# pycompression/python-zlib-ng

Measured on AMD Instinct MI355X. Metric: MB/s compress+decompress, 128 KiB blocks level 6, higher is better.
Workload: dtype u8

## Files before the change

python-zlib-ng_amd/csrc/za_deflate.hip:

```cpp
#include "za_common.h"
#include "za_crc.h"
#include <type_traits>

#define ZA_CH_GROUP 16
#define ZA_CH_OFFS(x) (((x) >> (32 - ZA_HASH_BITS - 2)) & (((1u << ZA_HASH_BITS) - 1u) << 2))
#define ZA_CH_CHUNK (64 * ZA_CH_GROUP)

typedef uint32_t za_v4u32 __attribute__((ext_vector_type(4)));
__device__ __forceinline__ void za_issue_load16(za_v4u32 &dst, const uint8_t *addr)
{
    asm volatile("global_load_dwordx4 %0, %1, off" : "=v"(dst) : "v"(addr) : "memory");
}
template <int NEWER>
__device__ __forceinline__ void za_wait_loads(za_v4u32 &a, za_v4u32 &b, za_v4u32 &c, za_v4u32 &d)
{
    asm volatile("s_waitcnt vmcnt(%4)" : "+v"(a), "+v"(b), "+v"(c), "+v"(d) : "n"(NEWER) : "memory");
}

__device__ __noinline__ uint32_t za_chains_fix(uint32_t h, uint32_t A, uint32_t old, bool ins)
{
    uint32_t near = 0, pre = 0xFFFFFFFFu;
    const int lane = za_lane();
    const unsigned long long insm = __ballot(ins);
    for (int j = 0; j < 64; j++) {
// ... 626 lines not shown
                if (dl != 0 && dl <= L.max_dist && best_len < nice) {
                    const uint32_t q = P - (uint32_t)dl;
                    const uint32_t sh = q & 3u;
                    const uint32_t *cw = (const uint32_t *)(lds + (q & (uint32_t)(ZA_BYTES - 4)));
                    const uint32_t c0 = cw[0], c1 = cw[1], c2 = cw[2], c3 = cw[3], c4 = cw[4];
                    const uint32_t x0 = __builtin_amdgcn_alignbyte(c1, c0, sh) ^ me0, x1 = __builtin_amdgcn_alignbyte(c2, c1, sh) ^ me1;
                    const uint32_t x2 = __builtin_amdgcn_alignbyte(c3, c2, sh) ^ me2, x3 = __builtin_amdgcn_alignbyte(c4, c3, sh) ^ me3;
                    uint32_t fbit, f1, f2, f3;
                    asm("v_ffbl_b32 %0, %4\n\tv_ffbl_b32 %1, %5\n\tv_ffbl_b32 %2, %6\n\tv_ffbl_b32 %3, %7\n\t"
                        "v_add_u32_e64 %1, %1, 32 clamp\n\tv_add_u32_e64 %2, %2, 64 clamp\n\tv_add_u32_e64 %3, %3, %8 clamp\n\t"
                        "v_min3_u32 %0, %0, %1, %2\n\tv_min_u32_e32 %0, %0, %3"
                        : "=&v"(fbit), "=&v"(f1), "=&v"(f2), "=&v"(f3) : "v"(x0), "v"(x1), "v"(x2), "v"(x3), "s"(96u));
                    int len = (int)min(fbit >> 3, 16u);
                    if (len == 16 && cap > 16) len = za_search_extend(win32, q, P, len, maxlen);
                    len = len < cap ? len : cap;
                    const bool better = len > best_len || (len == best_len && dl < best_dist);
                    best_len = better ? len : best_len;
                    best_dist = better ? dl : best_dist;
                }
            }
            uint32_t result = 0;
            if (best_len >= ZA_MIN_MATCH && !(best_len == 3 && best_dist > L.too_far3) && !(best_len == 4 && best_dist > L.too_far4))
                result = ((uint32_t)best_len << 15) | (uint32_t)(best_dist - 1);
            longm = longm || best_len > 64;
            best[p] = __builtin_amdgcn_perm(me0, result, 0x04020100u);
        };
        auto push = [&](bool alive, int p, uint32_t P, uint32_t q, int best_len, int best_dist, int depth) {
            const unsigned long long m = __ballot(alive);
            if (alive) {
                const uint32_t at = wl_n + __builtin_amdgcn_mbcnt_hi((uint32_t)(m >> 32), __builtin_amdgcn_mbcnt_lo((uint32_t)m, 0u));
                wl[2 * at] = (uint32_t)(p - base) | ((uint32_t)best_len << 12) | ((uint32_t)depth << 21);
                wl[2 * at + 1] = (P - q) | ((uint32_t)best_dist << 16);
            }
            wl_n += (uint32_t)__builtin_popcountll(m);
            __builtin_amdgcn_fence(__ATOMIC_RELEASE, "wavefront");
            __builtin_amdgcn_wave_barrier();
        };
        auto batch = [&](uint32_t nb) {
            wl_n -= nb;
            const bool has = (uint32_t)lane < nb;
            uint32_t e0 = 0, e1 = 0;
            __builtin_amdgcn_fence(__ATOMIC_ACQUIRE, "wavefront");
            if (has) { e0 = wl[2 * (wl_n + lane)]; e1 = wl[2 * (wl_n + lane) + 1]; }
            __builtin_amdgcn_fence(__ATOMIC_ACQ_REL, "wavefront");
            __builtin_amdgcn_wave_barrier();
            bool alive = false;
            int p = 0, best_len = 0, best_dist = 0, depth = 0;
            uint32_t P = 0, q = 0;
            if (has) {
                p = base + (int)(e0 & 0xFFFu);
                best_len = (int)((e0 >> 12) & 0x1FFu); depth = (int)(e0 >> 21); best_dist = (int)(e1 >> 16);
                P = goff + (uint32_t)(ZA_WIN + p);
                q = P - (e1 & 0xFFFFu);
                int seg_end = ((p >> sshift) + 1) << sshift;
                if (seg_end > n) seg_end = n;
                int maxlen = seg_end - p;
                if (maxlen > ZA_MAX_MATCH) maxlen = ZA_MAX_MATCH;
                const int cap = L.cap < maxlen ? L.cap : maxlen, nice = L.nice < cap ? L.nice : cap;
                uint32_t me0, me1, me2, me3;
                my16(P, me0, me1, me2, me3);
                const uint32_t sq = q % ZA_RING;
                uint32_t qb = RING_B0 + 2u * sq;
                uint32_t d = *(const uint16_t *)(lds + qb);
                alive = visit(P, me0, me1, me2, me3, maxlen, cap, nice, q, qb, d, best_len, best_dist, depth);
                if (!alive) finish(p, P, me0, me1, me2, me3, maxlen, cap, nice, best_len, best_dist, (uint32_t)linkb[p], USEC ? (uint32_t)linkc[p] : 0u);
            }
            push(alive, p, P, q, best_len, best_dist, depth);
        };
        uint32_t slot = (goff + (uint32_t)(ZA_WIN + base + tid)) % ZA_RING;
        load_own_links(base + ZA_SEARCH_TILE);
#pragma unroll
        for (int k = 0; k < ZA_SEARCH_TILE / ZA_SEARCH_THREADS; k++, slot = slot + ZA_SEARCH_THREADS >= ZA_RING ? slot + ZA_SEARCH_THREADS - ZA_RING : slot + ZA_SEARCH_THREADS) {
            const int p = base + k * ZA_SEARCH_THREADS + tid;
            bool alive = false;
            const uint32_t P = goff + (uint32_t)(ZA_WIN + p);
            uint32_t q = P;
            int best_len = ZA_MIN_MATCH - 1, best_dist = 0, depth = L.chain;
            if (p < n) {
                int seg_end = ((p >> sshift) + 1) << sshift;
                if (seg_end > n) seg_end = n;
                int maxlen = seg_end - p;
                if (maxlen > ZA_MAX_MATCH) maxlen = ZA_MAX_MATCH;
                uint32_t me0, me1, me2, me3;
                my16(P, me0, me1, me2, me3);
                const int cap = L.cap < maxlen ? L.cap : maxlen, nice = L.nice < cap ? L.nice : cap;
                if (maxlen >= ZA_MIN_MATCH) {
                    uint32_t qb = RING_B0 + 2u * slot;
                    uint32_t d = *(const uint16_t *)(lds + qb);
                    alive = visit(P, me0, me1, me2, me3, maxlen, cap, nice, q, qb, d, best_len, best_dist, depth);
                }
                if (!alive) finish(p, P, me0, me1, me2, me3, maxlen, cap, nice, best_len, best_dist, lkb[k], lkc[k]);
            }
            push(alive, p, P, q, best_len, best_dist, depth);
            while (__builtin_amdgcn_readfirstlane((int)wl_n) >= 64) batch(64u);
        }
        for (;;) {
            const uint32_t left = (uint32_t)__builtin_amdgcn_readfirstlane((int)wl_n);
            if (left == 0) break;
            batch(left < 64u ? left : 64u);
        }
        } else {
        uint32_t slot = (goff + (uint32_t)(ZA_WIN + base + (CONSEC ? 4 * tid : tid))) % ZA_RING;
        load_own_links(base + ZA_SEARCH_TILE);
        if (stats && base > 0) stats_issue(base - ZA_SEARCH_TILE);
#ifndef ZA_SEARCH_KUNROLL
#define ZA_SEARCH_KUNROLL 4
#endif
        const int p0c = base + 4 * tid;
        const uint32_t P0c = goff + (uint32_t)(ZA_WIN + p0c);
        uint32_t cm0 = 0, cm1 = 0, cm2 = 0, cm3 = 0, cm4 = 0;
        uint2 cdq = make_uint2(0u, 0u);
        int cseg_end = 0;
        if (CONSEC && p0c < n) {
            const uint32_t w = (P0c & (ZA_BYTES - 1)) >> 2;
            cm0 = win32[w]; cm1 = win32[w + 1]; cm2 = win32[w + 2]; cm3 = win32[w + 3]; cm4 = win32[w + 4];
            cdq = *(const uint2 *)(lds + RING_B0 + 2u * slot);
            cseg_end = ((p0c >> sshift) + 1) << sshift;
            if (cseg_end > n) cseg_end = n;
        }
#pragma unroll
        for (int k = 0; k < ZA_SEARCH_TILE / ZA_SEARCH_THREADS; k++, slot = CONSEC ? slot : slot + ZA_SEARCH_THREADS >= ZA_RING ? slot + ZA_SEARCH_THREADS - ZA_RING : slot + ZA_SEARCH_THREADS) {
            const int p = CONSEC ? p0c + k : base + k * ZA_SEARCH_THREADS + tid;
            res[k] = 0u;
            if (p >= n) continue;
            int seg_end = cseg_end;
            if (!CONSEC) {
                seg_end = ((p >> sshift) + 1) << sshift;
                if (seg_end > n) seg_end = n;
            }
            int maxlen = seg_end - p;
            if (maxlen > ZA_MAX_MATCH) maxlen = ZA_MAX_MATCH;
            uint32_t result = 0;
            const uint32_t P = goff + (uint32_t)(ZA_WIN + p);
            uint32_t me0, me1, me2, me3;
            if (CONSEC) {
                if (k == 0) { me0 = cm0; me1 = cm1; me2 = cm2; me3 = cm3; }
                else {
                    me0 = __builtin_amdgcn_alignbyte(cm1, cm0, (uint32_t)k); me1 = __builtin_amdgcn_alignbyte(cm2, cm1, (uint32_t)k);
                    me2 = __builtin_amdgcn_alignbyte(cm3, cm2, (uint32_t)k); me3 = __builtin_amdgcn_alignbyte(cm4, cm3, (uint32_t)k);
                }
            } else {
                const uint32_t idx = P & (ZA_BYTES - 1), w = idx >> 2, sh = idx & 3u;
                const uint32_t m0 = win32[w], m1 = win32[w + 1], m2 = win32[w + 2], m3 = win32[w + 3], m4 = win32[w + 4];
                me0 = __builtin_amdgcn_alignbyte(m1, m0, sh); me1 = __builtin_amdgcn_alignbyte(m2, m1, sh);
                me2 = __builtin_amdgcn_alignbyte(m3, m2, sh); me3 = __builtin_amdgcn_alignbyte(m4, m3, sh);
            }
            if (maxlen >= ZA_MIN_MATCH) {
                const int cap = L.cap < maxlen ? L.cap : maxlen;
                const int nice = L.nice < cap ? L.nice : cap;
                int best_len = ZA_MIN_MATCH - 1, best_dist = 0;
                uint32_t q = P;
                uint32_t qb = RING_B0 + 2u * (CONSEC ? slot + (uint32_t)k : slot);
                uint32_t d = CONSEC ? ((k < 2 ? cdq.x : cdq.y) >> (16 * (k & 1))) & 0xFFFFu : (uint32_t)*(const uint16_t *)(lds + qb);
                int depth = STEPS > 0 ? STEPS : L.chain;
#pragma unroll
                while (depth-- > 0) {
                    q -= d;
                    qb -= 2u * d;
                    qb += qb < RING_B0 ? RING_BYTES : 0u;
                    const int dist = (int)(P - q);
                    if (dist > L.max_dist) break;
                    d = *(const uint16_t *)(lds + qb);
                    const uint32_t sh = q & 3u;
                    const uint32_t *cw = (const uint32_t *)(lds + (q & (uint32_t)(ZA_BYTES - 4)));
                    const uint32_t c0 = cw[0], c1 = cw[1], c2 = cw[2], c3 = cw[3], c4 = cw[4];
                    uint32_t x0 = __builtin_amdgcn_alignbyte(c1, c0, sh) ^ me0;
                    uint32_t x1 = __builtin_amdgcn_alignbyte(c2, c1, sh) ^ me1;
                    uint32_t x2 = __builtin_amdgcn_alignbyte(c3, c2, sh) ^ me2;
                    uint32_t x3 = __builtin_amdgcn_alignbyte(c4, c3, sh) ^ me3;
                    uint32_t fbit, f1, f2, f3;
                    asm("v_ffbl_b32 %0, %4\n\tv_ffbl_b32 %1, %5\n\tv_ffbl_b32 %2, %6\n\tv_ffbl_b32 %3, %7\n\t"
                        "v_add_u32_e64 %1, %1, 32 clamp\n\tv_add_u32_e64 %2, %2, 64 clamp\n\tv_add_u32_e64 %3, %3, %8 clamp\n\t"
                        "v_min3_u32 %0, %0, %1, %2\n\tv_min_u32_e32 %0, %0, %3"
                        : "=&v"(fbit), "=&v"(f1), "=&v"(f2), "=&v"(f3) : "v"(x0), "v"(x1), "v"(x2), "v"(x3), "s"(96u));
                    int len = (int)min(fbit >> 3, FULL ? 16u : (uint32_t)cap);
                    if (FULL && len == 16 && cap > 16 && best_len < cap &&
                        (best_len < 16 || (uint8_t)za_lds_ld32(win32, q + (uint32_t)best_len) == (uint8_t)za_lds_ld32(win32, P + (uint32_t)best_len))) {
                        len = za_search_extend(win32, q, P, len, maxlen);
                    }
                    if (FULL) len = len < cap ? len : cap;
                    const bool better = len > best_len;
                    best_len = better ? len : best_len;
                    best_dist = better ? dist : best_dist;
                    if (best_len >= nice) break;
                }
                bool from_bc = false;
#ifndef ZA_ABL_SEARCH_NO_B
                {
                    const uint32_t dl = lkb[k];
#ifdef ZA_ABL_BC_SELF
                    const uint32_t q2 = P - (dl & 3u);
#else
                    const uint32_t q2 = P - dl;
#endif
                    const uint32_t *cw = (const uint32_t *)(lds + (q2 & (uint32_t)(ZA_BYTES - 4)));
                    const uint32_t c0 = cw[0], c1 = cw[1];
                    const uint32_t x = (__builtin_amdgcn_alignbyte(c1, c0, q2 & 3u) ^ me0) << 8;
                    const bool better = x == 0u && dl != 0u && (int)dl <= L.max_dist &&
                                        (ZA_HASH_BYTES_B > best_len || (ZA_HASH_BYTES_B == best_len && (int)dl < best_dist));
                    best_len = better ? ZA_HASH_BYTES_B : best_len;
                    best_dist = better ? (int)dl : best_dist;
                    from_bc = better;
                }
#endif
#ifndef ZA_ABL_SEARCH_NO_C
                if (USEC) {
                    const uint32_t dl = lkc[k];
#ifdef ZA_ABL_BC_SELF
                    const uint32_t q2 = P - (dl & 3u);
#else
                    const uint32_t q2 = P - dl;
#endif
                    const uint32_t sh = q2 & 3u;
                    const uint32_t *cw = (const uint32_t *)(lds + (q2 & (uint32_t)(ZA_BYTES - 4)));
                    const uint32_t c0 = cw[0], c1 = cw[1], c2 = cw[2], c3 = cw[3];
                    const uint32_t x = (__builtin_amdgcn_alignbyte(c1, c0, sh) ^ me0) | (__builtin_amdgcn_alignbyte(c2, c1, sh) ^ me1) |
                                       (__builtin_amdgcn_alignbyte(c3, c2, sh) ^ me2);
                    const bool better = x == 0u && dl != 0u && (int)dl <= L.max_dist && cap >= ZA_HASH_BYTES_C &&
                                        (ZA_HASH_BYTES_C > best_len || (ZA_HASH_BYTES_C == best_len && (int)dl < best_dist));
                    best_len = better ? ZA_HASH_BYTES_C : best_len;
                    best_dist = better ? (int)dl : best_dist;
                    from_bc = from_bc || better;
                }
#endif
#ifndef ZA_ABL_NO_EXTEND
                if (!FULL && (best_len == cap || from_bc) && best_len < maxlen) {
                    best_len = za_search_extend(win32, P - (uint32_t)best_dist, P, best_len, maxlen);
                }
#endif
                if (best_len >= ZA_MIN_MATCH && !(best_len == 3 && best_dist > L.too_far3) && !(best_len == 4 && best_dist > L.too_far4))
                    result = ((uint32_t)best_len << 15) | (uint32_t)(best_dist - 1);
                longm = longm || best_len > 64;
            }
#ifdef ZA_ABL_SEARCH_NOLIT
            res[k] = result;
#else
            res[k] = __builtin_amdgcn_perm(me0, result, 0x04020100u);
#endif
        }
        res_base = base;
        }
        if (pq < need_links) store_quad(pq, need_links, nq);
        {
            const int p = bytes_loaded + 8 * tid;
            if (p < need_bytes) {
                const uint64_t v = nbv >> nsh;
                store_bytes(p, (uint32_t)v);
                if (p + 4 < need_bytes) store_bytes(p + 4, (uint32_t)(v >> 32));
            }
        }
        if (ZA_OWN_STAGE) own_store(base + ZA_SEARCH_TILE);
        links_loaded = need_links; bytes_loaded = need_bytes;
        if (stats) { flush_results(); stats_use(); __syncthreads(); }
        else za_lds_barrier();
    }
    if constexpr (!FULL) flush_results();
    if (stats && n > 0) {
        __syncthreads();
        stats_issue((n - 1) & ~(ZA_SEARCH_TILE - 1));
        stats_use();
        for (int d = 32; d >= 1; d >>= 1) { st_U += (uint32_t)__shfl_xor((int)st_U, d, 64); st_NM += (uint32_t)__shfl_xor((int)st_NM, d, 64); }
        if ((tid & 63) == 0) { atomicAdd(&st_cnt[0], st_U); atomicAdd(&st_cnt[1], st_NM); }
        __syncthreads();
        const uint32_t U = st_cnt[0], NM = st_cnt[1];
        uint32_t hh = 0u;
        if (tid < 256) {
            hh = 16u * st_hist[tid] + 1u + (U >> 6);
            st_hist[tid] = 0u;
            uint32_t T = hh;
            for (int d = 32; d >= 1; d >>= 1) T += (uint32_t)__shfl_xor((int)T, d, 64);
            if ((tid & 63) == 0) atomicAdd(&st_cnt[2], T);
        }
        __syncthreads();
        if (tid < 256) {
            const uint32_t T = st_cnt[2];
            uint32_t *cost = cost_ws + (size_t)ui * ZA_DP_COSTS;
            int lbias = za_ilog4(U + NM, U ? U : 1u), mbias = za_ilog4(U + NM, NM ? NM : 1u);
            lbias = lbias > 24 ? 24 : lbias;
            mbias = mbias > 24 ? 24 : mbias;
            const int cl = za_ilog4(T, hh) + lbias;
            cost[tid] = (uint32_t)(cl < 12 ? 12 : cl > 52 ? 52 : cl);
            if (tid == 0) { cost[256] = (uint32_t)(12 + mbias + 20); cost[257] = 0u; }
        }
        __syncthreads();
        if (tid < 4) st_cnt[tid] = 0u;
        st_U = 0u; st_NM = 0u;
    }
    if (L.dp && __ballot(longm) != 0ull && (tid & 63) == 0) cost_ws[(size_t)ui * ZA_DP_COSTS + 258] = 1u;
    carry_bytes = bytes_loaded; n_prev = n;
    }
}

#define ZA_PCH 32
#define ZA_PROW (ZA_PCH + 1)
#ifndef ZA_DP_NEAR
#define ZA_DP_NEAR   64
#endif
#define ZA_DP_ROWS   (ZA_DP_NEAR / 2 + 4)
#ifndef ZA_DCH
#define ZA_DCH       16
#endif
#define ZA_DROW      (ZA_DCH + 1)
#define ZA_DPIECES   (ZA_DCH / 4)
#define ZA_DP_SEGSLOTS 2064

__global__ __launch_bounds__(256) void za_k_dpstats(const ZaUnit *__restrict__ units, const uint32_t *__restrict__ best_ws,
                                                    uint32_t *__restrict__ cost_ws )
{
    __shared__ uint32_t hist[256];
    __shared__ uint32_t cnt[3], tsum;
    const int n = (int)units[blockIdx.x].in_len;
    const int tid = (int)threadIdx.x, lane = tid & 63;
    const uint32_t *best = best_ws + (size_t)blockIdx.x * ZA_BEST_STRIDE;
    hist[tid] = 0;
    if (tid < 3) cnt[tid] = 0;
    if (tid == 0) tsum = 0;
    __syncthreads();
    uint32_t U = 0, NM = 0;
    for (int base = 1024 * (tid >> 6); base < n; base += 4096) {
        const int i0 = base + 4 * lane;
        uint4 v = make_uint4(0u, 0u, 0u, 0u);
        uint32_t pv = 0;
        if (i0 < n) v = *(const uint4 *)(best + i0);
        if (lane == 0 && i0 > 0 && i0 < n) pv = best[i0 - 1];
        const uint32_t e[4] = {v.x, v.y, v.z, v.w};
        uint32_t lp = (uint32_t)__shfl_up((int)ZA_ELEN(v.w), 1, 64);
        if (lane == 0) lp = ZA_ELEN(pv);
#pragma unroll
        for (int k = 0; k < 4; k++) {
            const uint32_t len = ZA_ELEN(e[k]);
            if (i0 + k < n) {
                if (len == 0u || (len == 3u && ZA_EDIST(e[k]) > (uint32_t)ZA_DP_WEAK_DIST)) { atomicAdd(&hist[e[k] >> 24], 1u); U++; }
                else if (len + 1u != lp) NM++;
            }
            lp = len;
        }
    }
    for (int d = 32; d >= 1; d >>= 1) { U += (uint32_t)__shfl_xor((int)U, d, 64); NM += (uint32_t)__shfl_xor((int)NM, d, 64); }
    if (lane == 0) { atomicAdd(&cnt[0], U); atomicAdd(&cnt[1], NM); }
    __syncthreads();
    U = cnt[0]; NM = cnt[1];
    const uint32_t hh = 16u * hist[tid] + 1u + (U >> 6);
    uint32_t T = hh;
    for (int d = 32; d >= 1; d >>= 1) T += (uint32_t)__shfl_xor((int)T, d, 64);
    if (lane == 0) atomicAdd(&tsum, T);
    __syncthreads();
    T = tsum;
    uint32_t *cost = cost_ws + (size_t)blockIdx.x * ZA_DP_COSTS;
    if (n == 0) return;
    int lbias = za_ilog4(U + NM, U ? U : 1u), mbias = za_ilog4(U + NM, NM ? NM : 1u);
    lbias = lbias > 24 ? 24 : lbias;
    mbias = mbias > 24 ? 24 : mbias;
    const int c = za_ilog4(T, hh) + lbias;
    cost[tid] = (uint32_t)(c < 12 ? 12 : c > 52 ? 52 : c);
    if (tid == 0) { cost[256] = (uint32_t)(12 + mbias + 20); cost[257] = 0u; }
}

__device__ __forceinline__ uint32_t za_pk_add_u16(uint32_t a, uint32_t b)
{
    uint32_t r;
    asm("v_pk_add_u16 %0, %1, %2" : "=v"(r) : "v"(a), "v"(b));
    return r;
}

__global__ __launch_bounds__(64) void za_k_optparse(const ZaUnit *__restrict__ units, uint32_t *__restrict__ best_ws,
                                                    const uint32_t *__restrict__ cost_ws, uint32_t *__restrict__ tok_ws ,
                                                    ZaLevel L)
{
    __shared__ uint32_t costt[ZA_DP_COSTS + 4];
    __shared__ uint32_t xt[3 * (ZA_MAX_MATCH + 1)];
    __shared__ uint32_t ring[ZA_DP_ROWS * 64];
    __shared__ uint32_t rowb[64 * ZA_DROW];
#ifndef ZA_DP_PAD
#define ZA_DP_PAD 2304
#endif
#if ZA_DP_PAD > 0
    __shared__ uint32_t dp_pad[ZA_DP_PAD / 4];
    if (units[blockIdx.x].in_len == 0xFFFFFFFFu) {
        dp_pad[threadIdx.x] = blockIdx.x; __syncthreads(); best_ws[threadIdx.x] = dp_pad[(threadIdx.x * 7u + best_ws[0]) % (ZA_DP_PAD / 4)];
    }
#endif
    const ZaUnit u = units[blockIdx.x];
    const int n = (int)u.in_len;
    const int lane = za_lane();
    const int sshift = ZA_UNIT_SEG_SHIFT(u.flags), seg = 1 << sshift;
    const int nseg = (n + seg - 1) >> sshift;
    uint32_t *best = best_ws + (size_t)blockIdx.x * ZA_BEST_STRIDE;
    if (n == 0) return;
    for (int i = lane; i < ZA_DP_COSTS; i += 64) costt[i] = cost_ws[(size_t)blockIdx.x * ZA_DP_COSTS + i];
    if (L.fixed_cost) {
        __syncthreads();
        for (int i = lane; i < 256; i += 64) costt[i] = i < 144 ? 32u : 36u;
        if (lane == 0) costt[256] = 48u;
    }
    for (int len = lane; len <= ZA_MAX_MATCH; len += 64) {
        const int l0 = len > 7 ? len - ZA_DP_SUB : 3;
        uint32_t x[ZA_DP_SUB + 1];
#pragma unroll
        for (int k = 0; k <= ZA_DP_SUB; k++) {
            const int l = l0 + k;
            int lc, ln = 0, le;
            if (l <= ZA_MAX_MATCH) za_len_sym(l, lc, ln, le);
            x[k] = (len >= 3 && l <= len && l >= L.min_len) ? (uint32_t)(4 * ln) : 0x3FFFu;
        }
        xt[3 * len] = x[0] | (x[1] << 16); xt[3 * len + 1] = x[2] | (x[3] << 16); xt[3 * len + 2] = x[4] | ((uint32_t)l0 << 16);
    }
    for (int i = lane; i < ZA_DP_ROWS * 64; i += 64) ring[i] = 0;
    __syncthreads();

    const int s0 = lane << sshift;
    int s1 = s0 + seg;
    if (s1 > n) s1 = n;
    const bool active = lane < nseg;
    uint32_t *myb = rowb + lane * ZA_DROW;
    uint8_t *myring = (uint8_t *)(ring + lane);
    uint16_t *accg = (uint16_t *)(tok_ws + (size_t)blockIdx.x * ZA_TOK_STRIDE) + (size_t)lane * ZA_DP_SEGSLOTS;
    auto ring_put = [&](int slot, uint32_t v) {
        *(uint16_t *)(myring + (slot >> 1) * 256 + (slot & 1) * 2) = (uint16_t)v;
        if (slot < 8) *(uint16_t *)(myring + ((slot >> 1) + ZA_DP_NEAR / 2) * 256 + (slot & 1) * 2) = (uint16_t)v;
    };
    const int mbase = (int)costt[256];
#ifdef ZA_ABL_DP_NOLONG
    const bool has_long = false;
#else
    const bool has_long = costt[258] != 0u;
#endif
    if (active) { ring_put((s1 - s0) & (ZA_DP_NEAR - 1), 0u); accg[s1 - s0] = 0; }
    int acc_next = 0;
    int far_base = -100;
    uint32_t fw[8] = {0u, 0u, 0u, 0u, 0u, 0u, 0u, 0u};
    uint4 pb[ZA_DPIECES];
    auto prefetch = [&](int c) {
#pragma unroll
        for (int j = 0; j < ZA_DPIECES; j++) {
            const int sg = (64 / ZA_DPIECES) * j + lane / ZA_DPIECES, off = (sg << sshift) + c * ZA_DCH + 4 * (lane % ZA_DPIECES);
            pb[j] = make_uint4(0, 0, 0, 0);
            if (c >= 0 && sg < nseg && off < n) pb[j] = *(const uint4 *)(best + off);
        }
    };
    struct Fetch { uint32_t e, clit, x0, x1, x2, w0, w1, w2; };
    auto stage_b = [&](uint32_t e, int idx_p) -> Fetch {
        Fetch f;
        f.e = e;
        f.clit = costt[e >> 24];
        const uint32_t len = ZA_ELEN(e);
        const uint32_t *xr = xt + 3u * len;
        f.x0 = xr[0]; f.x1 = xr[1]; f.x2 = xr[2];
        const uint32_t l0 = len > 7u ? len - (uint32_t)ZA_DP_SUB : 3u;
        const uint32_t st = ((uint32_t)idx_p + l0) & (uint32_t)(ZA_DP_NEAR - 1);
        const uint8_t *rp = myring + (st >> 1) * 256;
        f.w0 = *(const uint32_t *)rp; f.w1 = *(const uint32_t *)(rp + 256); f.w2 = *(const uint32_t *)(rp + 512);
        return f;
    };
    const int nch = ((n < seg ? n : seg) + ZA_DCH - 1) / ZA_DCH;
    uint4 po[ZA_DPIECES];
    uint32_t wacc[ZA_DCH / 2];
    int pend = -1;
    auto flush_pending = [&](auto longs_tag) {
        if (pend < 0) return;
        const int pcb = s0 + pend * ZA_DCH;
        if (decltype(longs_tag)::value && active && pcb < s1) {
            uint4 *g = (uint4 *)(accg + pend * ZA_DCH);
#pragma unroll
            for (int k = 0; k < ZA_DCH / 8; k++) g[k] = make_uint4(wacc[4 * k], wacc[4 * k + 1], wacc[4 * k + 2], wacc[4 * k + 3]);
        }
#pragma unroll
        for (int j = 0; j < ZA_DPIECES; j++) {
            const int sg = (64 / ZA_DPIECES) * j + lane / ZA_DPIECES, off = (sg << sshift) + pend * ZA_DCH + 4 * (lane % ZA_DPIECES);
            if (sg < nseg && off < n) *(uint4 *)(best + off) = po[j];
        }
    };
    prefetch(nch - 1);
    auto walk = [&](auto longs_tag) {
    constexpr bool LONGS = decltype(longs_tag)::value;
#pragma unroll 1
    for (int c = nch - 1; c >= 0; c--) {
        const int cb = s0 + c * ZA_DCH;
        __builtin_amdgcn_wave_barrier();
#pragma unroll
        for (int j = 0; j < ZA_DPIECES; j++) {
            uint32_t *r = rowb + ((64 / ZA_DPIECES) * j + lane / ZA_DPIECES) * ZA_DROW + 4 * (lane % ZA_DPIECES);
            r[0] = pb[j].x; r[1] = pb[j].y; r[2] = pb[j].z; r[3] = pb[j].w;
        }
        __builtin_amdgcn_fence(__ATOMIC_RELEASE, "wavefront");
        __builtin_amdgcn_wave_barrier();
        __builtin_amdgcn_fence(__ATOMIC_ACQUIRE, "wavefront");
        flush_pending(longs_tag);
        prefetch(c - 1);
        if (__ballot(active && cb < s1) != 0ull) {
            const int ib = c * ZA_DCH;
            uint32_t e_a = myb[ZA_DCH - 2];
            Fetch f = stage_b(myb[ZA_DCH - 1], ib + ZA_DCH - 1);
#pragma unroll 4
            for (int j = ZA_DCH - 1; j >= 0; j--) {
                const int idx = ib + j;
                const bool live = active && cb + j < s1;
                const Fetch g = f;
                if (j >= 1) f = stage_b(e_a, idx - 1);
                if (j >= 2) e_a = myb[j - 2];
                const uint32_t e = g.e, len = ZA_ELEN(e), dm1 = e & 0x7FFFu, l0 = g.x2 >> 16;
                const uint32_t st1 = ((uint32_t)idx + l0) & 1u;
                uint32_t v0 = __builtin_amdgcn_alignbyte(g.w1, g.w0, 2u * st1), v1 = __builtin_amdgcn_alignbyte(g.w2, g.w1, 2u * st1);
                uint32_t v2 = st1 ? g.w2 >> 16 : g.w2;
                if (LONGS && __builtin_expect(__ballot(live && len > (uint32_t)ZA_DP_NEAR) != 0ull, 0)) {
                    if (live && len > (uint32_t)ZA_DP_NEAR) {
                        const int e_lo = idx + (int)len - ZA_DP_SUB;
                        if (e_lo < far_base || e_lo + ZA_DP_SUB > far_base + 15) {
                            far_base = (e_lo + ZA_DP_SUB - 14) & ~1;
                            __builtin_amdgcn_fence(__ATOMIC_ACQ_REL, "workgroup");
                            const uint32_t *g32 = (const uint32_t *)(accg + far_base);
#pragma unroll
                            for (int k = 0; k < 8; k++) fw[k] = __hip_atomic_load(g32 + k, __ATOMIC_RELAXED, __HIP_MEMORY_SCOPE_AGENT);
                        }
                        const uint32_t o = (uint32_t)(e_lo - far_base), q = o >> 1;
                        uint32_t w0 = fw[0], w1 = fw[1], w2 = fw[2];
#pragma unroll
                        for (uint32_t k = 1; k <= 5; k++) { w0 = q == k ? fw[k] : w0; w1 = q == k ? fw[k + 1] : w1; w2 = q == k ? fw[k + 2] : w2; }
                        const uint32_t sh = (o & 1u) * 2u;
                        v0 = __builtin_amdgcn_alignbyte(w1, w0, sh); v1 = __builtin_amdgcn_alignbyte(w2, w1, sh);
                        v2 = (o & 1u) ? w2 >> 16 : w2;
                    }
                }
                int de = 30 - (int)__builtin_clz(dm1 | 1u);
                de = de < 0 ? 0 : de;
                const uint32_t b16 = (uint32_t)(mbase + 4 * de - acc_next) & 0xFFFFu;
                const uint32_t bb = b16 | (b16 << 16);
                uint32_t sA = za_pk_add_u16(za_pk_add_u16(v0, g.x0), bb);
                const uint32_t sB = za_pk_add_u16(za_pk_add_u16(v1, g.x1), bb);
                const uint32_t sC = za_pk_add_u16(za_pk_add_u16(v2, g.x2), bb);
                if (l0 == 3u && dm1 >= (uint32_t)L.too_far3) sA = (sA & 0xFFFF0000u) | 0x3FFFu;
#ifdef ZA_DP_TAGS_SHIFT
                const int t0 = (__builtin_amdgcn_sbfe((int)sA, 0, 16) << 3) | 4, t1 = (((int)sA >> 16) << 3) | 3;
                const int t2 = (__builtin_amdgcn_sbfe((int)sB, 0, 16) << 3) | 2, t3 = (((int)sB >> 16) << 3) | 1;
                const int t4 = __builtin_amdgcn_sbfe((int)sC, 0, 16) << 3;
#else
                int t0, t1, t2, t3, t4;
                asm("v_mad_i32_i16 %0, %5, 8, 4\n\tv_mad_i32_i16 %1, %5, 8, 3 op_sel:[1,0,0,0]\n\t"
                    "v_mad_i32_i16 %2, %6, 8, 2\n\tv_mad_i32_i16 %3, %6, 8, 1 op_sel:[1,0,0,0]\n\tv_mad_i32_i16 %4, %7, 8, 0"
                    : "=&v"(t0), "=&v"(t1), "=&v"(t2), "=&v"(t3), "=&v"(t4) : "v"(sA), "v"(sB), "v"(sC));
#endif
                int t = t0 < t1 ? t0 : t1;
                t = t < t2 ? t : t2;
                int tb = t3 < t4 ? t3 : t4;
                t = t < tb ? t : tb;
                const int mc = t >> 3;
                const bool ok = mc < (int)g.clit;
                const int c_best = ok ? mc : (int)g.clit;
                const uint32_t choice = ok ? l0 + 4u - ((uint32_t)t & 7u) : 0u;
                if (live) {
                    acc_next += c_best;
                    ring_put(idx & (ZA_DP_NEAR - 1), (uint32_t)acc_next);
                    myb[j] = (e & (ok ? 0xFF007FFFu : 0xFF000000u)) | (choice << 15);
                }
            }
        }
        __builtin_amdgcn_fence(__ATOMIC_RELEASE, "wavefront");
        __builtin_amdgcn_wave_barrier();
        __builtin_amdgcn_fence(__ATOMIC_ACQUIRE, "wavefront");
        if (LONGS && active && cb < s1) {
            const uint8_t *rp = myring + ((c * ZA_DCH) & (ZA_DP_NEAR - 1)) / 2 * 256;
#pragma unroll
            for (int k = 0; k < ZA_DCH / 2; k++) wacc[k] = *(const uint32_t *)(rp + 256 * k);
        }
#pragma unroll
        for (int j = 0; j < ZA_DPIECES; j++) {
            const uint32_t *r = rowb + ((64 / ZA_DPIECES) * j + lane / ZA_DPIECES) * ZA_DROW + 4 * (lane % ZA_DPIECES);
            po[j] = make_uint4(r[0], r[1], r[2], r[3]);
        }
        pend = c;
    }
    flush_pending(longs_tag);
    };
    if (has_long) walk(std::true_type{}); else walk(std::false_type{});
}

template <bool FILT> __device__ __forceinline__ uint32_t za_minlen(uint32_t lf, const ZaLevel &L)
{
    return (!FILT || lf >= (uint32_t)L.min_len) ? lf : 0u;
}



template <bool FILT>
__global__ __launch_bounds__(64) void za_k_parse(const ZaUnit *__restrict__ units,
                                                 const uint32_t *__restrict__ best_ws, uint32_t *__restrict__ tok_ws,
                                                 uint32_t *__restrict__ segtok_ws, uint32_t *__restrict__ hist_ws,
                                                 uint32_t *__restrict__ crc_out,
                                                 const uint32_t *__restrict__ crc_table,
                                                 const uint32_t *__restrict__ x8k_table,
                                                 ZaLevel L)
{
    __shared__ uint32_t hist[ZA_HIST_STRIDE];
    __shared__ uint32_t crct[256];
    __shared__ uint32_t rowb[64 * ZA_PROW + 3];
    const ZaUnit u = units[blockIdx.x];
    const int n = (int)u.in_len;
    const int lane = za_lane();
    const int sshift = ZA_UNIT_SEG_SHIFT(u.flags), seg = 1 << sshift;
    const int nseg = (n + seg - 1) >> sshift;
    for (int i = lane; i < ZA_HIST_STRIDE; i += 64) hist[i] = 0;
    for (int i = lane; i < 256; i += 64) crct[i] = crc_table[i];
    __syncthreads();

    const int s0 = lane << sshift;
    int s1 = s0 + seg;
    if (s1 > n) s1 = n;
    const bool active = lane < nseg;
    const uint32_t *best = best_ws + (size_t)blockIdx.x * ZA_BEST_STRIDE;
    uint32_t *myb = rowb + lane * ZA_PROW;

    uint4 pb[8];
    auto prefetch = [&](int c) {
        const int rel = c * ZA_PCH;
#pragma unroll
        for (int j = 0; j < 8; j++) {
            const int sg = 8 * j + (lane >> 3), off = (sg << sshift) + rel;
            pb[j] = make_uint4(0, 0, 0, 0);
            if (c < seg / ZA_PCH && sg < nseg && off < n) {
                typedef uint32_t za_v4u __attribute__((ext_vector_type(4)));
                const za_v4u v = __builtin_nontemporal_load((const za_v4u *)(best + off + 4 * (lane & 7)));
                pb[j] = make_uint4(v.x, v.y, v.z, v.w);
            }
        }
    };

    uint32_t ntok = 0;
    uint32_t crc_r = 0xFFFFFFFFu;
    int p = s0;
    uint32_t carry_b = 0;
    uint32_t nchunk = 0;
    prefetch(0);
#pragma unroll 1
    for (int c = 0; c < seg / ZA_PCH; c++) {
        const int cb = s0 + c * ZA_PCH;
        if (__ballot(active && cb < s1) == 0ull) break;
        __builtin_amdgcn_wave_barrier();
#pragma unroll
        for (int j = 0; j < 8; j++) {
            uint32_t *r = rowb + (8 * j + (lane >> 3)) * ZA_PROW + 1 + 4 * (lane & 7);
            r[0] = pb[j].x; r[1] = pb[j].y; r[2] = pb[j].z; r[3] = pb[j].w;
        }
        myb[0] = carry_b;
        __builtin_amdgcn_wave_barrier();
        prefetch(c + 1);
        int ce = cb + ZA_PCH;
        if (ce > s1) ce = s1;
        if (active && cb < s1) {
#ifndef ZA_ABL_PARSE_NOCRC
            {
                int k = cb;
                for (; k + 4 <= ce; k += 4) {
                    const uint32_t *e = myb + 1 + (k - cb);
                    const uint32_t w4 = __builtin_amdgcn_perm(e[1], e[0], 0x0c0c0703u) | __builtin_amdgcn_perm(e[3], e[2], 0x07030c0cu);
                    crc_r = crct[(crc_r ^ w4) & 0xFF] ^ (crc_r >> 8);
                    crc_r = crct[(crc_r ^ (w4 >> 8)) & 0xFF] ^ (crc_r >> 8);
                    crc_r = crct[(crc_r ^ (w4 >> 16)) & 0xFF] ^ (crc_r >> 8);
                    crc_r = crct[(crc_r ^ (w4 >> 24)) & 0xFF] ^ (crc_r >> 8);
                }
                for (; k < ce; k++) crc_r = crct[(crc_r ^ (myb[1 + k - cb] >> 24)) & 0xFF] ^ (crc_r >> 8);
            }
#endif
            {
                const int lim = ce == s1 ? ce : ce - 1;
                auto push = [&](uint32_t t) {
                    myb[nchunk] = t;
                    nchunk++;
                };
                while (p < lim) {
                    const uint32_t b = myb[p - cb + 1], bn = myb[p - cb + 2], e2 = myb[p - cb + 3];
                    const uint32_t lf = za_minlen<FILT>(ZA_ELEN(b), L), nlf = za_minlen<FILT>(ZA_ELEN(bn), L);
                    const bool is_match = lf != 0u;
                    const int len = (int)lf;
                    const uint32_t lit = b >> 24;
                    const int dist = is_match ? (int)ZA_EDIST(b) : 1;
                    int lc, ln, le, dc, dn, de;
                    za_len_sym(is_match ? len : 3, lc, ln, le);
                    za_dist_sym(dist, dc, dn, de);
                    const bool c1 = lf == 0u && p + 1 < ce && nlf == 0u;
                    const bool c2 = c1 && p + 2 < ce && za_minlen<FILT>(ZA_ELEN(e2), L) == 0u;
                    const uint32_t l1 = bn >> 24, l2 = e2 >> 24;
                    const uint32_t t = is_match ? (0x80000000u | ((uint32_t)lc << 26) | ((uint32_t)le << 21) | ((uint32_t)dc << 16) | (uint32_t)de)
                                                : lit | (c1 ? l1 << 8 : 0u) | (c2 ? l2 << 16 : 0u) | (((c1 ? 1u : 0u) + (c2 ? 1u : 0u)) << 24);
                    push(t);
#ifndef ZA_ABL_PARSE_NOHIST
                    atomicAdd(&hist[is_match ? 257u + (uint32_t)lc : lit], 1u);
                    if (is_match) atomicAdd(&hist[288 + dc], 1u);
                    if (c1) atomicAdd(&hist[l1], 1u);
                    if (c2) atomicAdd(&hist[l2], 1u);
#endif
                    p += is_match ? len : 1 + (c1 ? 1 : 0) + (c2 ? 1 : 0);
                }
            }
            carry_b = myb[ZA_PCH];
        }
        __builtin_amdgcn_fence(__ATOMIC_RELEASE, "wavefront");
        __builtin_amdgcn_wave_barrier();
#pragma unroll
        for (int j = 0; j < 8; j++) {
            const int sg = 8 * j + (lane >> 3);
            const uint32_t cnt = (uint32_t)__shfl((int)nchunk, sg, 64), at = (uint32_t)__shfl((int)ntok, sg, 64);
            const uint32_t first = 4u * (uint32_t)(lane & 7);
            const uint32_t *r = rowb + sg * ZA_PROW;
            uint32_t *dst = tok_ws + (size_t)blockIdx.x * ZA_TOK_STRIDE + ((size_t)sg << sshift) + at;
            if (first < cnt) {
                if (at + first + 4u <= (uint32_t)seg) { ZaU4u v; v.x = r[first]; v.y = r[first + 1]; v.z = r[first + 2]; v.w = r[first + 3]; *(ZaU4u *)(dst + first) = v; }
                else for (uint32_t i = first; i < cnt && i < first + 4u; i++) dst[i] = r[i];
            }
            if ((lane & 7) == 7 && cnt > 32u) dst[32] = r[32];
        }
        ntok += nchunk; nchunk = 0;
        __builtin_amdgcn_wave_barrier();
    }
    uint32_t cseg = 0;
    if (active) {
        cseg = crc_r ^ 0xFFFFFFFFu;
        if (lane < nseg - 1) {
            const int tail = n - ((nseg - 1) << sshift);
            uint32_t xt = 0x80000000u, sq = 0x00800000u;
            for (int m = tail; m; m >>= 1) { if (m & 1) xt = za_multmodp(sq, xt); sq = za_multmodp(sq, sq); }
            uint32_t xk = 0x80000000u;
            if (sshift == ZA_SEG_SHIFT) xk = x8k_table[nseg - 2 - lane];
            else {
                uint32_t xs = 0x00800000u;
                for (int i = 0; i < sshift; i++) xs = za_multmodp(xs, xs);
                for (int m = nseg - 2 - lane; m; m >>= 1) { if (m & 1) xk = za_multmodp(xs, xk); xs = za_multmodp(xs, xs); }
            }
            cseg = za_multmodp(za_multmodp(xk, xt), cseg);
        }
    }
    cseg = za_wave_xor_reduce(cseg);
    if (lane == 0) crc_out[blockIdx.x] = cseg;
    segtok_ws[(size_t)blockIdx.x * ZA_MAX_SEGS + lane] = ntok;
    __syncthreads();
    if (lane == 0) hist[256] = 1;
    __syncthreads();
    for (int i = lane; i < ZA_HIST_STRIDE; i += 64) hist_ws[(size_t)blockIdx.x * ZA_HIST_STRIDE + i] = hist[i];
}

#define ZA_RCH 64
#define ZA_RROW (ZA_RCH / 4 + 1)
#define ZA_RTOK 68
#define ZA_RTROW (ZA_RTOK + 1)
template <bool RUNS>
__global__ __launch_bounds__(64) void za_k_parse_rle(const uint8_t *__restrict__ in, const ZaUnit *__restrict__ units,
                                                     uint32_t *__restrict__ tok_ws, uint32_t *__restrict__ segtok_ws,
                                                     uint32_t *__restrict__ hist_ws, uint32_t *__restrict__ crc_out,
                                                     const uint32_t *__restrict__ crc_table,
                                                     const uint32_t *__restrict__ x8k_table)
{
    __shared__ uint32_t hist[ZA_HIST_STRIDE];
    __shared__ uint32_t crct[256];
    __shared__ uint32_t rowb[64 * ZA_RROW];
    __shared__ uint32_t tokb[64 * ZA_RTROW];
    const ZaUnit u = units[blockIdx.x];
    const int n = (int)u.in_len;
    const int lane = za_lane();
    const int sshift = ZA_UNIT_SEG_SHIFT(u.flags), seg = 1 << sshift;
    const int nseg = (n + seg - 1) >> sshift;
    for (int i = lane; i < ZA_HIST_STRIDE; i += 64) hist[i] = 0;
    for (int i = lane; i < 256; i += 64) crct[i] = crc_table[i];
    __syncthreads();

    const uint8_t *ub = in + u.in_off;
    const int s0 = lane << sshift;
    int s1 = s0 + seg;
    if (s1 > n) s1 = n;
    const bool active = lane < nseg;
    const int sh = (int)((uintptr_t)(ub + s0) & 15u);
    const int rend = active ? sh + (s1 - s0) : 0;
    const uint32_t *myrow = rowb + lane * ZA_RROW;
    uint32_t *mytok = tokb + lane * ZA_RTROW;

    typedef uint32_t za_v4u __attribute__((ext_vector_type(4)));
    za_v4u pb[4];
    auto prefetch = [&](int c) {
#pragma unroll
        for (int j = 0; j < 4; j++) {
            const int sg = 16 * j + (lane >> 2);
            pb[j] = za_v4u{0u, 0u, 0u, 0u};
            if (sg < nseg) {
                const uint8_t *first = ub + (sg << sshift);
                const int send = ((sg + 1) << sshift) < n ? ((sg + 1) << sshift) : n;
                const uint8_t *a = (const uint8_t *)((uintptr_t)first & ~(uintptr_t)15) + c * ZA_RCH + 16 * (lane & 3);
                if (a < ub + send) pb[j] = __builtin_nontemporal_load((const za_v4u *)a);
            }
        }
    };

    uint32_t crc_r = 0xFFFFFFFFu;
    uint32_t ntok = 0, nchunk = 0;
    uint32_t litw = 0, litn = 0;
    uint32_t prev = 0x100u, pend = 0;
    if (RUNS && active && (s0 > 0 || u.dict_len > 0)) prev = ub[s0 - 1];
    bool done = !active;
    auto push = [&](uint32_t t) { mytok[nchunk] = t; nchunk++; };
    auto lit = [&](uint32_t b) {
        litw |= b << (8u * litn);
        atomicAdd(&hist[b], 1u);
        if (++litn == 3u) { push(litw | (2u << 24)); litw = 0; litn = 0; }
    };
    auto flush_lits = [&]() { if (litn) { push(litw | ((litn - 1u) << 24)); litw = 0; litn = 0; } };
    auto match = [&](uint32_t len) {
        flush_lits();
        int lc, ln, le;
        za_len_sym((int)len, lc, ln, le);
        push(0x80000000u | ((uint32_t)lc << 26) | ((uint32_t)le << 21));
        atomicAdd(&hist[257 + lc], 1u);
        atomicAdd(&hist[288], 1u);
    };
    auto close_run = [&]() {
        if (pend >= 3u) match(pend);
        else for (uint32_t k = 0; k < pend; k++) lit(prev);
        pend = 0;
    };

    const int nch = (15 + (n < seg ? n : seg) + ZA_RCH - 1) / ZA_RCH;
    prefetch(0);
#pragma unroll 1
    for (int c = 0; c < nch; c++) {
        const int ib = c * ZA_RCH;
        if (__ballot(ib < rend) == 0ull) break;
        __builtin_amdgcn_wave_barrier();
#pragma unroll
        for (int j = 0; j < 4; j++) {
            uint32_t *r = rowb + (16 * j + (lane >> 2)) * ZA_RROW + 4 * (lane & 3);
            r[0] = pb[j].x; r[1] = pb[j].y; r[2] = pb[j].z; r[3] = pb[j].w;
        }
        __builtin_amdgcn_wave_barrier();
        prefetch(c + 1);
        if (ib < rend) {
#pragma unroll 2
            for (int k = 0; k < ZA_RCH / 4; k++) {
                const uint32_t w = myrow[k];
#pragma unroll
                for (int b = 0; b < 4; b++) {
                    const int i = ib + 4 * k + b;
                    if (i >= sh && i < rend) {
                        const uint32_t x = (w >> (8 * b)) & 0xFFu;
                        crc_r = crct[(crc_r ^ x) & 0xFFu] ^ (crc_r >> 8);
                        if (RUNS && x == prev) {
                            if (++pend == (uint32_t)ZA_MAX_MATCH) { match(pend); pend = 0; }
                        } else {
                            if (RUNS) { close_run(); prev = x; }
                            lit(x);
                        }
                    }
                }
            }
        }
        if (!done && rend <= ib + ZA_RCH) {
            if (RUNS) close_run();
            flush_lits();
            done = true;
        }
        __builtin_amdgcn_fence(__ATOMIC_RELEASE, "wavefront");
        __builtin_amdgcn_wave_barrier();
#pragma unroll
        for (int j = 0; j < 8; j++) {
            const int sg = 8 * j + (lane >> 3);
            const uint32_t cnt = (uint32_t)__shfl((int)nchunk, sg, 64), at = (uint32_t)__shfl((int)ntok, sg, 64);
            const uint32_t *r = tokb + sg * ZA_RTROW;
            uint32_t *dst = tok_ws + (size_t)blockIdx.x * ZA_TOK_STRIDE + ((size_t)sg << sshift) + at;
#pragma unroll
            for (int q = 0; q < 3; q++) {
                const uint32_t first = 4u * (uint32_t)((lane & 7) + 8 * q);
                if (first < cnt) {
                    if (at + first + 4u <= (uint32_t)seg) { ZaU4u v; v.x = r[first]; v.y = r[first + 1]; v.z = r[first + 2]; v.w = r[first + 3]; *(ZaU4u *)(dst + first) = v; }
                    else for (uint32_t i = first; i < cnt && i < first + 4u; i++) dst[i] = r[i];
                }
            }
        }
        ntok += nchunk; nchunk = 0;
        __builtin_amdgcn_wave_barrier();
    }
// ... 770 lines not shown
```

Before: 59000.

## Move optimal-parse best entries in 128-byte lines of two chunks

The backward DP walk in za_k_optparse now loads and stores the per-position best entries in rounds of 32 positions (two 16-entry chunks), so each lane group touches a full 128-byte line per global access rather than a 64-byte half. The upper chunk is staged into LDS right away and the lower one is held in registers for the next iteration. Write-back is deferred until both chunks of a round are done. This aims to improve global memory coalescing and cut transaction count, at the cost of extra registers (plo/ohi/pb/po doubled) that may lower occupancy.

Result: no change. 59270, median of 6 (+0.5%).

```diff
diff --git a/python-zlib-ng_amd/csrc/za_deflate.hip b/python-zlib-ng_amd/csrc/za_deflate.hip
--- a/python-zlib-ng_amd/csrc/za_deflate.hip
+++ b/python-zlib-ng_amd/csrc/za_deflate.hip
@@ -952,6 +952,15 @@
 #endif
 #define ZA_DROW      (ZA_DCH + 1)
 #define ZA_DPIECES   (ZA_DCH / 4)
+#ifndef ZA_DP_LINES
+#define ZA_DP_LINES  1
+#endif
+#define ZA_DGCH      (ZA_DP_LINES ? 2 : 1)
+#define ZA_DGR       (ZA_DGCH * ZA_DCH)
+#define ZA_DGPIECES  (ZA_DGR / 4)
+#if ZA_DP_LINES && ZA_DCH != 16
+#error "ZA_DP_LINES = 1 moves rounds of 32 positions as two chunks of 16"
+#endif
 #define ZA_DP_SEGSLOTS 2064
 
 __global__ __launch_bounds__(256) void za_k_dpstats(const ZaUnit *__restrict__ units, const uint32_t *__restrict__ best_ws,
@@ -1013,6 +1022,10 @@
     return r;
 }
 
+static_assert(ZA_BEST_STRIDE % 32 == 0, "a unit's rows of entries start at multiples of 128 bytes");
+#ifdef ZA_DP_WAVES_PER_SIMD
+__attribute__((amdgpu_waves_per_eu(ZA_DP_WAVES_PER_SIMD, ZA_DP_WAVES_PER_SIMD)))
+#endif
 __global__ __launch_bounds__(64) void za_k_optparse(const ZaUnit *__restrict__ units, uint32_t *__restrict__ best_ws,
                                                     const uint32_t *__restrict__ cost_ws, uint32_t *__restrict__ tok_ws ,
                                                     ZaLevel L)
@@ -1079,13 +1092,23 @@
     int acc_next = 0;
     int far_base = -100;
     uint32_t fw[8] = {0u, 0u, 0u, 0u, 0u, 0u, 0u, 0u};
-    uint4 pb[ZA_DPIECES];
-    auto prefetch = [&](int c) {
-#pragma unroll
-        for (int j = 0; j < ZA_DPIECES; j++) {
-            const int sg = (64 / ZA_DPIECES) * j + lane / ZA_DPIECES, off = (sg << sshift) + c * ZA_DCH + 4 * (lane % ZA_DPIECES);
+    uint4 pb[ZA_DGPIECES];
+    auto za_piece = [&](int j, int &sg) -> int {
+#if ZA_DP_LINES
+        sg = 16 * (j >> 1) + (lane >> 2);
+        return (sg << sshift) + (j & 1 ? 0 : ZA_DCH) + 4 * (lane & 3);
+#else
+        sg = (64 / ZA_DPIECES) * j + lane / ZA_DPIECES;
+        return (sg << sshift) + 4 * (lane % ZA_DPIECES);
+#endif
+    };
+    auto prefetch = [&](int r) {
+#pragma unroll
+        for (int j = 0; j < ZA_DGPIECES; j++) {
+            int sg;
+            const int off = za_piece(j, sg) + r * ZA_DGR;
             pb[j] = make_uint4(0, 0, 0, 0);
-            if (c >= 0 && sg < nseg && off < n) pb[j] = *(const uint4 *)(best + off);
+            if (r >= 0 && sg < nseg && off < n) pb[j] = *(const uint4 *)(best + off);
         }
     };
     struct Fetch { uint32_t e, clit, x0, x1, x2, w0, w1, w2; };
@@ -1103,40 +1126,58 @@
         return f;
     };
     const int nch = ((n < seg ? n : seg) + ZA_DCH - 1) / ZA_DCH;
-    uint4 po[ZA_DPIECES];
+    const int nrd = (nch + ZA_DGCH - 1) / ZA_DGCH;
+    uint4 po[ZA_DGPIECES];
     uint32_t wacc[ZA_DCH / 2];
-    int pend = -1;
-    auto flush_pending = [&](auto longs_tag) {
+    int pend = -1, pend_acc = -1;
+    auto flush_acc = [&](auto longs_tag) {
+        if (decltype(longs_tag)::value && pend_acc >= 0 && active && s0 + pend_acc * ZA_DCH < s1) {
+            uint4 *g = (uint4 *)(accg + pend_acc * ZA_DCH);
+#pragma unroll
+            for (int k = 0; k < ZA_DCH / 8; k++) g[k] = make_uint4(wacc[4 * k], wacc[4 * k + 1], wacc[4 * k + 2], wacc[4 * k + 3]);
+        }
+    };
+    auto flush_pending = [&]() {
         if (pend < 0) return;
-        const int pcb = s0 + pend * ZA_DCH;
-        if (decltype(longs_tag)::value && active && pcb < s1) {
-            uint4 *g = (uint4 *)(accg + pend * ZA_DCH);
-#pragma unroll
-            for (int k = 0; k < ZA_DCH / 8; k++) g[k] = make_uint4(wacc[4 * k], wacc[4 * k + 1], wacc[4 * k + 2], wacc[4 * k + 3]);
-        }
-#pragma unroll
-        for (int j = 0; j < ZA_DPIECES; j++) {
-            const int sg = (64 / ZA_DPIECES) * j + lane / ZA_DPIECES, off = (sg << sshift) + pend * ZA_DCH + 4 * (lane % ZA_DPIECES);
+#pragma unroll
+        for (int j = 0; j < ZA_DGPIECES; j++) {
+            int sg;
+            const int off = za_piece(j, sg) + pend * ZA_DGR;
             if (sg < nseg && off < n) *(uint4 *)(best + off) = po[j];
         }
     };
-    prefetch(nch - 1);
+#if ZA_DP_LINES
+    uint4 plo[ZA_DPIECES], ohi[ZA_DPIECES];
+#endif
+    prefetch(nrd - 1);
     auto walk = [&](auto longs_tag) {
     constexpr bool LONGS = decltype(longs_tag)::value;
 #pragma unroll 1
-    for (int c = nch - 1; c >= 0; c--) {
+    for (int c = nrd * ZA_DGCH - 1; c >= 0; c--) {
         const int cb = s0 + c * ZA_DCH;
+        const bool top = ZA_DGCH == 1 || (c & 1);
         __builtin_amdgcn_wave_barrier();
-#pragma unroll
-        for (int j = 0; j < ZA_DPIECES; j++) {
+        auto stage = [&](int j, const uint4 &v) {
             uint32_t *r = rowb + ((64 / ZA_DPIECES) * j + lane / ZA_DPIECES) * ZA_DROW + 4 * (lane % ZA_DPIECES);
-            r[0] = pb[j].x; r[1] = pb[j].y; r[2] = pb[j].z; r[3] = pb[j].w;
-        }
+            r[0] = v.x; r[1] = v.y; r[2] = v.z; r[3] = v.w;
+        };
+#if ZA_DP_LINES
+        if (top) {
+#pragma unroll
+            for (int j = 0; j < ZA_DPIECES; j++) { stage(j, pb[2 * j]); plo[j] = pb[2 * j + 1]; }
+        } else {
+#pragma unroll
+            for (int j = 0; j < ZA_DPIECES; j++) stage(j, plo[j]);
+        }
+#else
+#pragma unroll
+        for (int j = 0; j < ZA_DPIECES; j++) stage(j, pb[j]);
+#endif
         __builtin_amdgcn_fence(__ATOMIC_RELEASE, "wavefront");
         __builtin_amdgcn_wave_barrier();
         __builtin_amdgcn_fence(__ATOMIC_ACQUIRE, "wavefront");
-        flush_pending(longs_tag);
-        prefetch(c - 1);
+        flush_acc(longs_tag);
+        if (top) { flush_pending(); prefetch(c / ZA_DGCH - 1); }
         if (__ballot(active && cb < s1) != 0ull) {
             const int ib = c * ZA_DCH;
             uint32_t e_a = myb[ZA_DCH - 2];
@@ -1212,14 +1253,28 @@
 #pragma unroll
             for (int k = 0; k < ZA_DCH / 2; k++) wacc[k] = *(const uint32_t *)(rp + 256 * k);
         }
-#pragma unroll
-        for (int j = 0; j < ZA_DPIECES; j++) {
+        pend_acc = c;
+        auto unstage = [&](int j) {
             const uint32_t *r = rowb + ((64 / ZA_DPIECES) * j + lane / ZA_DPIECES) * ZA_DROW + 4 * (lane % ZA_DPIECES);
-            po[j] = make_uint4(r[0], r[1], r[2], r[3]);
-        }
+            return make_uint4(r[0], r[1], r[2], r[3]);
+        };
+#if ZA_DP_LINES
+        if (top) {
+#pragma unroll
+            for (int j = 0; j < ZA_DPIECES; j++) ohi[j] = unstage(j);
+        } else {
+#pragma unroll
+            for (int j = 0; j < ZA_DPIECES; j++) { po[2 * j] = ohi[j]; po[2 * j + 1] = unstage(j); }
+            pend = c / ZA_DGCH;
+        }
+#else
+#pragma unroll
+        for (int j = 0; j < ZA_DPIECES; j++) po[j] = unstage(j);
         pend = c;
-    }
-    flush_pending(longs_tag);
+#endif
+    }
+    flush_acc(longs_tag);
+    flush_pending();
     };
     if (has_long) walk(std::true_type{}); else walk(std::false_type{});
 }
```
